# justinkay/coda

Hardware: AMD Instinct MI355X
Metric: acquisition_steps_per_sec (higher is better)
Workload: dtype fp32; 1 GPU; model=coda-eig, task=imagenet1k-scale, H_models=128, N_points=50000, C_classes=1000, prefilter_n=0, chunk_size=256, global_batch=50000, seq_len=1000, parallelism=single

## Files before the change

### coda_amd/ops/hip/pair.hip

```cpp

#include <climits>
#include <initializer_list>
#include <torch/extension.h>
#include <hip/hip_runtime.h>
#include <c10/hip/HIPStream.h>
#include <hip/hip_bfloat16.h>
#include "wave.h"

#define P_POINTS 256
#define BLOCK 256

namespace pairops {

typedef __bf16 bf16x8 __attribute__((ext_vector_type(8)));
typedef float f32x4 __attribute__((ext_vector_type(4)));
typedef _Float16 half4v __attribute__((ext_vector_type(4)));

__device__ __forceinline__ void
dsum_es_row(const _Float16* __restrict__ delta16,
            const float* __restrict__ dall,
            const int* __restrict__ pair_c,
            const int* __restrict__ pair_neg,
            const int* __restrict__ seg_off,
            const int* __restrict__ seg_h,
// ... 291 lines not shown
    for (int jt = 0; jt < JT; ++jt) {
        const int j = jt * 16 + row16;
        if (j >= twoH) continue;
        const int h = j >> 1, v = j & 1;
        const float mix = mixture0[h];
        const float pbb = pbest_before[(size_t)c * H + h];
#pragma unroll
        for (int r = 0; r < 4; ++r) {
            const int bit = (vmw[r][jt >> 2] >> (h & 31)) & 1;
            if (bit == v)
                pair_ent_acc(ent[r], mix, pic, acc[jt][r], inv[r], pbb);
        }
    }
#pragma unroll
    for (int r = 0; r < 4; ++r) {
        const float e = row16_reduce(ent[r]);
        if (row16 == 0) h_after[kbase + r] = e;
    }
    }
    (void)mstride;
}


template <int JT>
__global__ void __launch_bounds__(BLOCK2)
pair_gemm_pbn128_kernel(const hip_bfloat16* __restrict__ a16,
                        const hip_bfloat16* __restrict__ egw,
                        const unsigned* __restrict__ vmask,
                        const int* __restrict__ pair_c,
                        int W,
                        const int* __restrict__ grp_off,
                        const int* __restrict__ cls_grp_off,
                        const int* __restrict__ run_off,
                        const long long* __restrict__ y_t,
                        float* __restrict__ pm,
                        float* __restrict__ pinv,
                        int C, int H) {
    int g = blockIdx.x, a_row0 = 0;
    if (y_t != nullptr) {
        const long long y = y_t[0];
        if (y < 0 || y >= C) return;
        g += cls_grp_off[y];
        if (g >= cls_grp_off[y + 1]) return;
        a_row0 = run_off[y];
    }
    extern __shared__ char smem[];
    const int twoH = 2 * H;
    hip_bfloat16* b_lds = reinterpret_cast<hip_bfloat16*>(smem);

    const int t0 = grp_off[g], t1 = grp_off[g + 1];
    const int c = pair_c[t0 * 128];
    const int tid = threadIdx.x;
    const int wave = tid >> 6, lane = tid & 63;
    const int row16 = lane & 15;
    const int kgrp = lane >> 4;
    const hip_bfloat16* egw_c = egw + (size_t)c * twoH * P_POINTS;

    for (int t = tid; t < 2 * twoH; t += BLOCK2) {
        const int j = t >> 1, half = t & 1;
        const uint4* g = reinterpret_cast<const uint4*>(
            egw_c + (size_t)j * P_POINTS + half * 128);
        uint4* d = reinterpret_cast<uint4*>(
            reinterpret_cast<char*>(b_lds)
            + (size_t)j * BSTRIDE * 2 + half * 256);
#pragma unroll
        for (int i = 0; i < 16; ++i) d[i] = g[i];
    }
    __syncthreads();

    for (int tile = t0; tile < t1; ++tile) {
    const int k0 = tile * 128;
    f32x4 acc[JT];
#pragma unroll
    for (int jt = 0; jt < JT; ++jt) acc[jt] = {0.f, 0.f, 0.f, 0.f};

    const hip_bfloat16* arow =
        a16 + (size_t)(k0 - a_row0 + wave * 16 + row16) * P_POINTS;
#pragma unroll
    for (int kk = 0; kk < P_POINTS; kk += 32) {
        const bf16x8 afrag = *reinterpret_cast<const bf16x8*>(
            arow + kk + kgrp * 8);
#pragma unroll
        for (int jt = 0; jt < JT; ++jt) {
            const int j = jt * 16 + row16;
            bf16x8 bfrag = {};
            if (j < twoH)
                bfrag = *reinterpret_cast<const bf16x8*>(
                    b_lds + (size_t)j * BSTRIDE + kk + kgrp * 8);
            acc[jt] = __builtin_amdgcn_mfma_f32_16x16x32_bf16(
                afrag, bfrag, acc[jt], 0, 0, 0);
        }
    }

// ... 22 lines not shown
#pragma unroll
    for (int r = 0; r < 4; ++r)
        inv[r] = 1.0f / fmaxf(row16_reduce(tot[r]), 1e-30f);

#pragma unroll
    for (int jt = 0; jt < JT; ++jt) {
        const int j = jt * 16 + row16;
        if (j >= twoH) continue;
        const int h = j >> 1, v = j & 1;
#pragma unroll
        for (int r = 0; r < 4; ++r) {
            const int bit = (vmw[r][jt >> 2] >> (h & 31)) & 1;
            if (bit == v) pm[(size_t)(kbase + r) * H + h] = acc[jt][r];
        }
    }
#pragma unroll
    for (int r = 0; r < 4; ++r)
        if (row16 == 0) pinv[kbase + r] = inv[r];
    }
}


#define ECH 4

__global__ void __launch_bounds__(BLOCK)
pair_entropy_cached_kernel(const float* __restrict__ pm,
                           const float* __restrict__ pinv,
                           const unsigned* __restrict__ vmask,
                           const int* __restrict__ pair_c,
                           int W,
                           const float* __restrict__ pi_hat,
                           const float* __restrict__ pbest_before,
                           const float* __restrict__ mixture0,
                           float* __restrict__ h_after,
                           int H) {
    extern __shared__ char smem[];
    float* rows = reinterpret_cast<float*>(smem);
    float* mix_s = rows + 16 * H;
    float* pbb_s = mix_s + H;

    const int kb = blockIdx.x * (16 * ECH);
    const int c = pair_c[kb];
    const int tid = threadIdx.x;
    const int nv4 = 4 * H;
    const f32x4* g = reinterpret_cast<const f32x4*>(pm + (size_t)kb * H);
    const f32x4 zero4 = {0.f, 0.f, 0.f, 0.f};
    f32x4 nxt[3];
#pragma unroll
    for (int q = 0; q < 3; ++q)
        nxt[q] = tid + q * BLOCK < nv4 ? g[tid + q * BLOCK] : zero4;
    for (int h = tid; h < H; h += BLOCK) {
        mix_s[h] = mixture0[h];
        pbb_s[h] = pbest_before[(size_t)c * H + h];
    }
    const int pi = tid >> 4, l = tid & 15;
    const float pic = pi_hat[c];
    const float* row = rows + pi * H;
    const int twoH = 2 * H;
    const int JT = (twoH + 15) / 16;

#pragma unroll
    for (int ch = 0; ch < ECH; ++ch) {
        f32x4* d = reinterpret_cast<f32x4*>(rows);
#pragma unroll
        for (int q = 0; q < 3; ++q)
            if (tid + q * BLOCK < nv4) d[tid + q * BLOCK] = nxt[q];
        __syncthreads();
        if (ch + 1 < ECH) {
            const f32x4* gn = g + (size_t)(ch + 1) * nv4;
#pragma unroll
            for (int q = 0; q < 3; ++q)
                nxt[q] = tid + q * BLOCK < nv4 ? gn[tid + q * BLOCK]
                                               : zero4;
        }
        const int k = kb + ch * 16 + pi;
        const float inv = pinv[k];
        float ent = 0.f;
        unsigned vw = 0u;
        for (int jt = 0; jt < JT; ++jt) {
            const int j = jt * 16 + l;
            if ((jt & 3) == 0)
                vw = (jt >> 2) < W ? vmask[(size_t)k * W + (jt >> 2)] : 0u;
            if (j >= twoH) continue;
            const int h = j >> 1, v = j & 1;
            const int bit = (vw >> (h & 31)) & 1;
            if (bit == v)
                pair_ent_acc(ent, mix_s[h], pic, row[h], inv, pbb_s[h]);
        }
        const float e = row16_reduce(ent);
        if (l == 0) h_after[k] = e;
        __syncthreads();
    }
}

#define WSTRIDE 40

__global__ void __launch_bounds__(BLOCK)
pair_gemm_wide_kernel(const hip_bfloat16* __restrict__ a16,
                      const hip_bfloat16* __restrict__ egw,
                      const int* __restrict__ pair_c,
                      hip_bfloat16* __restrict__ mout,
                      int twoH) {
    extern __shared__ char smem[];
    hip_bfloat16* a_lds = reinterpret_cast<hip_bfloat16*>(smem);
    hip_bfloat16* b_lds = a_lds + 2 * 128 * WSTRIDE;

    const int k0 = blockIdx.x * 128;
    const int j0 = blockIdx.y * 128;
    const int c = pair_c[k0];
    const int tid = threadIdx.x;
    const int wave = tid >> 6, lane = tid & 63;
    const int row16 = lane & 15, kgrp = lane >> 4;
    const hip_bfloat16* egw_c = egw + (size_t)c * twoH * P_POINTS;
// ... 84 lines not shown
    float tot = 0.f;
    int i = 0;
    for (int h = lane; h < H; h += 64, ++i) {
        const int v = (vm[h >> 5] >> (h & 31)) & 1;
        val[i] = (float)mrow[2 * h + v];
        tot += val[i];
    }
    tot = wave_reduce_sum(tot);
    const float inv = 1.0f / fmaxf(tot, 1e-30f);
    const float pic = pi_hat[c];
    float ent = 0.f;
    i = 0;
    for (int h = lane; h < H; h += 64, ++i) {
        const float pb = val[i] * inv;
        const float mm = fmaxf(
            mixture0[h] + pic * (pb - pbest_before[(size_t)c * H + h]),
            1e-12f);
        ent += -mm * __log2f(mm);
    }
    ent = wave_reduce_sum(ent);
    if (lane == 0) h_after[k] = ent;
}

__global__ void __launch_bounds__(BLOCK)
pair_eig_finalize_kernel(const float* __restrict__ h_after,
                         const float* __restrict__ h_base,
                         const int* __restrict__ pair_c,
                         const int* __restrict__ cand_off,
                         const long long* __restrict__ cand_ck,
                         const long* __restrict__ cand_ids,
                         const float* __restrict__ adjusted,
                         const float* __restrict__ row_sums,
                         float H_before,
                         float* __restrict__ q,
                         int B, int C) {
    const int b = blockIdx.x * 4 + (threadIdx.x >> 6);
    if (b >= B) return;
    const int lane = threadIdx.x & 63;
    const long id = cand_ids[b];
    const float inv = 1.0f / fmaxf(row_sums[id], 1e-12f);
    const float* arow = adjusted + (size_t)id * C;
    float base = 0.f;
    int cc = lane * 4;
    for (; cc + 3 < C; cc += 256) {
        const float4 a = *reinterpret_cast<const float4*>(arow + cc);
        const float4 hb = *reinterpret_cast<const float4*>(h_base + cc);
        base += a.x * hb.x + a.y * hb.y + a.z * hb.z + a.w * hb.w;
    }
    for (; cc < C; ++cc) base += arow[cc] * h_base[cc];
    float corr = 0.f;
    const int s1 = cand_off[b + 1];
    for (int s = cand_off[b] + lane; s < s1; s += 64) {
        const long long pk = cand_ck[s];
        const int k = (int)(pk >> 32);
        const int c2 = (int)(pk & 0xffffffff);
        corr += arow[c2] * (h_after[k] - h_base[c2]);
    }
    (void)pair_c;
    const float tot = wave_reduce_sum(base + corr);
    if (lane == 0) q[b] = H_before - tot * inv;
}

__global__ void __launch_bounds__(BLOCK)
pair_entropy_wide_cls_kernel(const hip_bfloat16* __restrict__ m,
                             const int* __restrict__ cls,
                             const int* __restrict__ pair_b,
                             const int* __restrict__ pair_c,
                             const float* __restrict__ pi_hat,
                             const float* __restrict__ pbest_before,
                             const float* __restrict__ mixture0,
                             float* __restrict__ h_after,
                             int K, int H) {
    const int k = blockIdx.x * 4 + (threadIdx.x >> 6);
    if (k >= K) return;
    const int lane = threadIdx.x & 63;
    const int c = pair_c[k];
    const int b = pair_b[k];
    const hip_bfloat16* mrow = m + (size_t)k * 2 * H;

    float tot = 0.f;
    for (int h = lane; h < H; h += 64) {
        const int v = (b >= 0 && cls[(size_t)b * H + h] == c) ? 1 : 0;
        tot += (float)mrow[2 * h + v];
// ... 542 lines not shown
    TORCH_CHECK(grp.scalar_type() == torch::kInt32 && grp.is_contiguous()
                && grp.numel() >= 2, "grp must be the (G+1,) tile groups");
    const bool one_class = y_t_o.has_value();
    int nblk = grp.numel() - 1;
    const int* cgo = nullptr;
    const int* roff = nullptr;
    const long long* yp = nullptr;
    if (one_class) {
        TORCH_CHECK(cls_grp_off_o.has_value() && run_off_o.has_value(),
                    "one-class mode needs cls_grp_off and run_off");
        const torch::Tensor& y_t = *y_t_o;
        const torch::Tensor& cls_grp_off = *cls_grp_off_o;
        const torch::Tensor& run_off = *run_off_o;
        TORCH_CHECK(y_t.is_cuda() && y_t.scalar_type() == torch::kInt64
                    && y_t.numel() == 1, "y_t must be a (1,) int64 tensor");
        TORCH_CHECK(cls_grp_off.scalar_type() == torch::kInt32
                    && cls_grp_off.is_contiguous()
                    && cls_grp_off.numel() == C + 1
                    && run_off.scalar_type() == torch::kInt32
                    && run_off.is_contiguous()
                    && run_off.numel() == C + 1,
                    "cls_grp_off / run_off must be (C+1,) int32");
        TORCH_CHECK(max_grp >= 1 && max_grp <= nblk);
        nblk = (int)max_grp;
        cgo = cls_grp_off.data_ptr<int>();
        roff = run_off.data_ptr<int>();
        yp = reinterpret_cast<const long long*>(y_t.data_ptr<int64_t>());
    } else {
        TORCH_CHECK(a16.size(0) == K, "full build needs the (K, P) operand");
    }
    const size_t shmem = (size_t)2 * H * BSTRIDE * sizeof(hip_bfloat16);
    const int JT = (2 * H + 15) / 16;
    auto stream = c10::hip::getCurrentHIPStream();
    auto launch = [&](auto kern) {
        hipLaunchKernelGGL(kern, dim3(nblk), dim3(BLOCK2), shmem,
                           stream.stream(),
                           reinterpret_cast<const hip_bfloat16*>(
                               a16.data_ptr()),
                           reinterpret_cast<const hip_bfloat16*>(
                               egw.data_ptr()),
                           reinterpret_cast<const unsigned*>(
                               vmask.data_ptr<int>()),
                           pair_c.data_ptr<int>(), (int)vmask.size(1),
                           grp.data_ptr<int>(), cgo, roff, yp,
                           pm.data_ptr<float>(), pinv.data_ptr<float>(),
                           C, H);
    };
    if (JT <= 4) launch(pairops::pair_gemm_pbn128_kernel<4>);
    else if (JT <= 8) launch(pairops::pair_gemm_pbn128_kernel<8>);
    else if (JT <= 16) launch(pairops::pair_gemm_pbn128_kernel<16>);
    else launch(pairops::pair_gemm_pbn128_kernel<17>);
}

torch::Tensor pair_entropy_cached(torch::Tensor pm, torch::Tensor pinv,
                                  torch::Tensor vmask,
                                  torch::Tensor pair_c,
                                  torch::Tensor pi_hat,
                                  torch::Tensor pbest_before,
                                  torch::Tensor mixture0) {
    TORCH_CHECK(pm.is_cuda() && pm.dtype() == torch::kFloat32
                && pm.is_contiguous() && pm.dim() == 2);
    const int K = pm.size(0);
    const int H = pm.size(1);
    TORCH_CHECK(K % 128 == 0 && 2 * H <= 272,
                "pair cache covers the fused route only");
    TORCH_CHECK(pinv.is_contiguous() && pinv.numel() == K
                && pair_c.numel() == K && vmask.size(0) == K);
    TORCH_CHECK(mixture0.numel() == H && mixture0.is_contiguous()
                && pbest_before.is_contiguous()
                && pbest_before.size(1) == H
                && pi_hat.is_contiguous());
    auto h_after = torch::empty({K}, pi_hat.options());
    if (K == 0) return h_after;
    const size_t shmem = (size_t)18 * H * sizeof(float);
    auto stream = c10::hip::getCurrentHIPStream();
    hipLaunchKernelGGL(pairops::pair_entropy_cached_kernel,
                       dim3(K / (16 * ECH)), dim3(BLOCK), shmem,
                       stream.stream(),
                       pm.data_ptr<float>(), pinv.data_ptr<float>(),
                       reinterpret_cast<const unsigned*>(
                           vmask.data_ptr<int>()),
                       pair_c.data_ptr<int>(), (int)vmask.size(1),
                       pi_hat.data_ptr<float>(),
                       pbest_before.data_ptr<float>(),
                       mixture0.data_ptr<float>(),
                       h_after.data_ptr<float>(), H);
    return h_after;
}

torch::Tensor pair_eig_finalize(torch::Tensor h_after,
                                torch::Tensor h_base,
                                torch::Tensor pair_c,
                                torch::Tensor cand_off,
                                torch::Tensor cand_ck,
                                torch::Tensor cand_ids,
                                torch::Tensor adjusted,
                                torch::Tensor row_sums,
                                double H_before) {
    const int B = cand_ids.size(0);
    const int C = adjusted.size(1);
    TORCH_CHECK(h_base.is_contiguous() && h_base.size(0) == C);
    TORCH_CHECK(cand_ck.scalar_type() == torch::kInt64,
                "cand_ck must be the packed int64 hit table");
    TORCH_CHECK(cand_ids.is_contiguous() && cand_off.is_contiguous()
                && cand_ck.is_contiguous(),
                "finalize inputs must be contiguous");
    auto q = torch::empty({B}, adjusted.options());
    auto stream = c10::hip::getCurrentHIPStream();
    hipLaunchKernelGGL(pairops::pair_eig_finalize_kernel,
                       dim3((B + 3) / 4), dim3(BLOCK), 0, stream.stream(),
                       h_after.data_ptr<float>(),
                       h_base.data_ptr<float>(), pair_c.data_ptr<int>(),
                       cand_off.data_ptr<int>(),
                       reinterpret_cast<const long long*>(
                           cand_ck.data_ptr<int64_t>()),
                       cand_ids.data_ptr<long>(),
                       adjusted.data_ptr<float>(),
                       row_sums.data_ptr<float>(),
                       (float)H_before, q.data_ptr<float>(), B, C);
    return q;
}

void acq_select(torch::Tensor q0, torch::Tensor h0, torch::Tensor active,
                torch::Tensor qbuf, torch::Tensor out,
                torch::Tensor ties,
                c10::optional<torch::Tensor> topk_o,
                c10::optional<torch::Tensor> group_of_o,
                int64_t n_groups) {
    TORCH_CHECK(q0.is_cuda() && q0.dtype() == torch::kFloat32
                && q0.is_contiguous(), "q0 must be contiguous fp32");
    TORCH_CHECK(h0.dtype() == torch::kFloat32 && h0.numel() == 1);
    TORCH_CHECK(active.dtype() == torch::kBool && active.is_contiguous()
                && active.numel() == q0.numel());
    TORCH_CHECK(qbuf.dtype() == torch::kFloat32 && qbuf.is_contiguous()
                && qbuf.numel() == q0.numel());
    TORCH_CHECK(out.dtype() == torch::kFloat64 && out.is_contiguous()
                && out.numel() == 3);
    TORCH_CHECK(ties.dtype() == torch::kInt64 && ties.is_contiguous()
                && ties.numel() >= 2, "ties buffer too small");
    const int cap = ties.numel() - 1;
    const int B = q0.numel();
    const bool want_topk = topk_o.has_value() && topk_o->defined();
// ... 143 lines not shown
          pybind11::arg("vmask"), pybind11::arg("pair_c"),
          pybind11::arg("pi_hat"),
          pybind11::arg("pbest_before"), pybind11::arg("mixture0"),
          pybind11::arg("tile"), pybind11::arg("ablate") = 0,
          pybind11::arg("grp") = torch::Tensor());
    m.def("pair_gemm_entropy_cls", &pair_gemm_entropy_cls,
          "v3 wide-H pairing GEMM + cls-based entropy -> (K,)");
    m.def("pair_dsum_es_cls", &pair_dsum_es_cls,
          "pair A-operand of ONE class (id read on device) into the "
          "(max_run, P) scratch operand");
    m.def("pair_gemm_pbn", &pair_gemm_pbn,
          "pair-cache build (all groups) / one-class refresh: selected "
          "pairing masses pm (K, H) and inv (K,)",
          pybind11::arg("a16"), pybind11::arg("egw"),
          pybind11::arg("vmask"), pybind11::arg("pair_c"),
          pybind11::arg("grp"), pybind11::arg("pm"),
          pybind11::arg("pinv"),
          pybind11::arg("cls_grp_off") = pybind11::none(),
          pybind11::arg("run_off") = pybind11::none(),
          pybind11::arg("y_t") = pybind11::none(),
          pybind11::arg("max_grp") = 0);
    m.def("pair_entropy_cached", &pair_entropy_cached,
          "per-step entropy pass over the pair cache -> (K,), bit-equal "
          "to the fused 128-pair kernel");
    m.def("pair_eig_finalize", &pair_eig_finalize,
          "v3 per-candidate EIG assembly (deterministic) -> (B,)");
    m.def("acq_select", &acq_select,
          "fused acquisition epilogue: qbuf = active ? h0+q0 : -inf; "
          "out(f64[3]) = [masked max, first argmax, isclose tie count]; "
          "topk (K,) int64, when given, = the K best in rank order, one "
          "per group with group_of, -1 padded",
          pybind11::arg("q0"), pybind11::arg("h0"),
          pybind11::arg("active"), pybind11::arg("qbuf"),
          pybind11::arg("out"), pybind11::arg("ties"),
          pybind11::arg("topk") = pybind11::none(),
          pybind11::arg("group_of") = pybind11::none(),
          pybind11::arg("n_groups") = 0);
    m.def("mfma_probe", &mfma_probe,
          "16x16x32 bf16 MFMA fragment-layout probe");
}
```

### coda_amd/ops/hip/wave.h

```cpp
#pragma once

#include <hip/hip_runtime.h>

template <int CTRL, int ROW_MASK>
__device__ __forceinline__ int dpp_mov(int x) {
    return __builtin_amdgcn_update_dpp(0, x, CTRL, ROW_MASK, 0xf, true);
}

template <int CTRL, int ROW_MASK>
__device__ __forceinline__ float dpp_add(float x) {
    return x + __int_as_float(dpp_mov<CTRL, ROW_MASK>(__float_as_int(x)));
}

__device__ __forceinline__ float wave_inclusive_scan(float v) {
    v = dpp_add<0x111, 0xf>(v);
    v = dpp_add<0x112, 0xf>(v);
    v = dpp_add<0x114, 0xf>(v);
    v = dpp_add<0x118, 0xf>(v);
    v = dpp_add<0x142, 0xa>(v);
    v = dpp_add<0x143, 0xc>(v);
    return v;
}

__device__ __forceinline__ float wave_reduce_sum(float v) {
    return __int_as_float(__builtin_amdgcn_readlane(
        __float_as_int(wave_inclusive_scan(v)), 63));
}

__device__ __forceinline__ float row16_reduce(float v) {
    v = dpp_add<0x111, 0xf>(v);
    v = dpp_add<0x112, 0xf>(v);
    v = dpp_add<0x114, 0xf>(v);
    v = dpp_add<0x118, 0xf>(v);
    return __shfl(v, 15, 16);
}
```

### coda_amd/ops/pair.py

```python
from __future__ import annotations

from typing import NamedTuple, Optional

import torch

from .reference import EPS_PROB, PBEST_NUM_POINTS

PAIR_TILE = 16


def tile_for(H: int, B: int) -> int:
    return 128 if B >= 4096 else PAIR_TILE


class PairStructure(NamedTuple):
    cand_ids: torch.Tensor
    pair_b: torch.Tensor
    pair_c: torch.Tensor
    seg_off: torch.Tensor
    seg_h: torch.Tensor
    base_pos: torch.Tensor
    n_real: int
    tile: int
    cand_off: torch.Tensor = None
    cand_pairs: torch.Tensor = None
    vmask: torch.Tensor = None
    pair_neg: torch.Tensor = None
    cand_ck: torch.Tensor = None
    grp_off: torch.Tensor = None
    cls_grp_off: torch.Tensor = None
    run_off: torch.Tensor = None
    max_grp: int = 0
    max_run: int = 0

    @property
    def K(self) -> int:
        return self.pair_b.shape[0]


def build_pairs(cls_rows: torch.Tensor, cand_ids: torch.Tensor,
                C: int, tile: int = 0,
                with_vmask: bool = True,
                dedupe: bool = True) -> PairStructure:
    device = cls_rows.device
    B, H = cls_rows.shape
    tile = tile or tile_for(H, B)
    cls_l = cls_rows.long()
    keys = (cls_l * B + torch.arange(B, device=device).unsqueeze(1))
    flat = keys.reshape(-1)
    order = torch.argsort(flat, stable=True)
    sk = flat[order]
    is_new = torch.ones_like(sk, dtype=torch.bool)
    is_new[1:] = sk[1:] != sk[:-1]
    pair_key = sk[is_new]
    pr_c = pair_key // B
    pr_b = pair_key - pr_c * B
# ... 81 lines not shown
    h1 = entry_h[mask1]
    if bool(flip_real[reps_idx].any()):
        flipped_reps = reps_idx[flip_real[reps_idx]]
        pair_neg[pos[new_of_u[uid_of_real[flipped_reps]]]] = 1
        q_of_b = torch.full((B,), -1, dtype=torch.long, device=device)
        q_of_b[pr_b[flipped_reps]] = flipped_reps
        entry_b = pr_b[entry_pid]
        qb = q_of_b[entry_b]
        comp = (qb >= 0) & (entry_pid != qb)
        t2 = pos[new_of_u[uid_of_real[qb[comp]]]]
        h2 = entry_h[comp]
        tgt = torch.cat([t1, t2])
        hh = torch.cat([h1, h2])
    else:
        tgt, hh = t1, h1
    srt = torch.argsort(tgt * H + hh)
    seg_h = hh[srt].to(torch.int32)
    seg_len_k = torch.bincount(tgt, minlength=K)
    seg_off = torch.zeros(K + 1, dtype=torch.int32, device=device)
    seg_off[1:] = seg_len_k.cumsum(0).to(torch.int32)

    grp_off = None
    if tile == 128 and K % 128 == 0 and K > 0:
        GRP_MAX = 4
        tc = pair_c[::128]
        T = tc.numel()
        newc = torch.ones(T, dtype=torch.bool, device=device)
        newc[1:] = tc[1:] != tc[:-1]
        idx = torch.arange(T, device=device)
        run_start = idx[newc]
        run_id = newc.long().cumsum(0) - 1
        off_in_run = idx - run_start[run_id]
        gstart = newc | (off_in_run % GRP_MAX == 0)
        grp_off = torch.cat([
            idx[gstart].to(torch.int32),
            torch.tensor([T], dtype=torch.int32, device=device),
        ]).contiguous()
        grp_per_cls = torch.bincount(tc[gstart].long(), minlength=C)
        cls_grp_off = torch.zeros(C + 1, dtype=torch.int32, device=device)
        cls_grp_off[1:] = grp_per_cls.cumsum(0).to(torch.int32)
        per_class = dict(cls_grp_off=cls_grp_off,
                         run_off=run_off.to(torch.int32),
                         max_grp=int(grp_per_cls.max()),
                         max_run=int(run_len.max()))
    else:
        per_class = {}

    return PairStructure(**per_class,
                         cand_ids=cand_ids.long().contiguous(),
                         pair_b=pair_b,
                         pair_c=pair_c, seg_off=seg_off, seg_h=seg_h,
                         base_pos=run_off[:-1].clone(), n_real=K2,
                         tile=tile, cand_off=cand_off,
                         cand_pairs=cand_pairs, vmask=vmask,
                         pair_neg=pair_neg, grp_off=grp_off,
                         cand_ck=((cand_pairs.long() << 32)
                                  | pair_c[cand_pairs.long()].long())
                         .contiguous() if cand_pairs is not None
                         else None)


def pair_pbn(tables, ps: PairStructure, cls_rows: torch.Tensor,
             k0: int = 0, k1: Optional[int] = None) -> torch.Tensor:
    EG, delta, s_base, w = (tables.EG, tables.delta, tables.s_base,
                            tables.weights)
    C, H, _, P = EG.shape
    k1 = ps.K if k1 is None else k1
# ... 104 lines not shown
    if cache.pbn is not None:
        y = int(y)
        k0, k1 = int(ps.run_off[y]), int(ps.run_off[y + 1])
        cache.pbn[k0:k1] = pair_pbn(tables, ps, cls_rows, k0, k1)
        return
    import coda_amd.ops as O
    O._ext.pair_dsum_es_cls(tables.delta16, tables.dall, ps.pair_c,
                            ps.pair_neg, ps.seg_off, ps.seg_h,
                            ps.run_off, y, cache.a_run)
    O._ext.pair_gemm_pbn(cache.a_run, tables.egw, ps.vmask, ps.pair_c,
                         ps.grp_off, cache.pm, cache.pinv,
                         ps.cls_grp_off, ps.run_off, y, ps.max_grp)


def pair_cache_h_after(cache: PairCache, ps: PairStructure,
                       pi_hat: torch.Tensor, pbest_before: torch.Tensor,
                       mixture0: torch.Tensor) -> torch.Tensor:
    if cache.pbn is not None:
        return h_after_from_pbn(cache.pbn, ps, pi_hat, pbest_before,
                                mixture0)
    import coda_amd.ops as O
    return O._ext.pair_entropy_cached(
        cache.pm, cache.pinv, ps.vmask, ps.pair_c, pi_hat.contiguous(),
        pbest_before.contiguous(), mixture0.contiguous())


def eig_from_pairs(h_after: torch.Tensor, ps: PairStructure,
                   adjusted: torch.Tensor, row_sums: torch.Tensor,
                   H_before) -> torch.Tensor:
    N = adjusted.shape[0]
    h_base = h_after[ps.base_pos]
    inv_rs = 1.0 / row_sums.clamp_min(1e-12)
    base_n = (adjusted @ h_base) * inv_rs
    counts = (ps.cand_off[1:] - ps.cand_off[:-1]).long()
    ids = torch.repeat_interleave(ps.cand_ids, counts)
    k = ps.cand_pairs.long()
    c_v = ps.pair_c[k].long()
    pix = adjusted[ids, c_v] * inv_rs[ids]
    corr = torch.zeros(N, device=adjusted.device)
    corr.index_add_(0, ids, pix * (h_after[k] - h_base[c_v]))
    if torch.is_tensor(H_before):
        H_before = H_before.to(base_n.dtype)
    return H_before - base_n - corr


def _h_after_kernels(tables, ps: PairStructure, cls_rows, pbest_before,
                     pi_hat, mixture0) -> torch.Tensor:
# ... 76 lines not shown
```

### coda_amd/selectors/coda.py

```python
from __future__ import annotations

import random

import torch
from sortedcontainers import SortedList

from ..base import ModelSelector
from ..parallel import Comm, get_comm
from .. import ops
from ..ops import pair as pops
from ..ops import sharded as shops
from ..ops import table as tops
from ..util import DEBUG, _check, mirror_fits
from .pair_acq import PairAcquisition, tied_choice

import os
DEBUG_VIZ = os.environ.get("CODA_AMD_DEBUG_VIZ") == "1"

_ON_DEVICE = object()


def _warm_and_capture(body, read=None):
    side = torch.cuda.Stream()
    side.wait_stream(torch.cuda.current_stream())
# ... 111 lines not shown
        self.q_vals = []
        self.stochastic = False
        self.step = 0
        self.reset_derived_state()
        self.update_pi_hat()

    def reset_derived_state(self):
        self._tables = None
        self._tables_dirty = set()
        self._pair_acq = None
        self._posterior_version = 0
        self._pbest_rows_cache = (-1, None)
        self._drop_graphs()
        self._merged_acq = False
        self._g_idx = self._g_y = self._g_pi = self._g_rows = None
        self._alpha_g, self._beta_g = self._gather_global_betas()
        self._active_candidates = SortedList(
            i for i in self.unlabeled_idxs if self._disagreement_host[i])

    def _drop_graphs(self):
        self._label_graph = None
        self._acq_graph = None
        self._acq_pending = None

    def _gather_global_betas(self):
        if not self._replicated:
            return None, None
        a_l, b_l = ops.dirichlet_to_beta(self.dirichlets)
        sizes = self.comm.shard_sizes(self.H)
        order = self.comm.unshard_order(self.H).to(self.device)
        return tuple(self.comm.all_gather_cat(
            t, dim=0, sizes=sizes)[order].contiguous() for t in (a_l, b_l))

    @classmethod
    def from_args(cls, dataset, args, comm=None):
        return cls(dataset,
                   prefilter_n=args.prefilter_n,
                   alpha=args.alpha,
                   learning_rate=args.learning_rate,
                   multiplier=args.multiplier,
                   disable_diag_prior=args.no_diag_prior,
                   q=args.q,
                   comm=comm,
                   chunk_size=getattr(args, "chunk_size", 100),
                   pi_hat_precision=getattr(args, "pi_hat_precision",
                                            "auto"))
# ... 216 lines not shown
                    hsizes=self.comm.shard_sizes(self.H))
            elif self.comm.is_distributed:
                eig = shops.eig_chunk_sharded(
                    alpha_cc, beta_cc, chunk_classes, pbest_before,
                    self.pi_hat, pi_xi, mixture0, H_before, self.comm,
                    num_points=self.num_points)
            elif tables is not None:
                eig = tops.eig_chunk_table(
                    tables, chunk_classes, pbest_before, self.pi_hat,
                    pi_xi, mixture0, H_before)
            else:
                eig = ops.eig_chunk(
                    alpha_cc, beta_cc, chunk_classes, pbest_before,
                    self.pi_hat, pi_xi, mixture0, H_before,
                    num_points=self.num_points)
            eig_chunks.append(eig)

        return torch.cat(eig_chunks), candidate_ids

    def _acq_body(self):
        acq = self._pair_acq
        rows, pi = self._g_rows, self._g_pi
        mixture0, H0 = ops.mixture_entropy(rows, pi)
        h_after = None if acq.cache is None else pops.pair_cache_h_after(
            acq.cache, acq.ps, pi, rows, mixture0)
        q0 = pops.eig_pairs(self._tables, acq.ps, acq.cls_rows, rows, pi,
                            mixture0, None, self._adjusted, self._row_sums,
                            h_after=h_after)
        ops._ext.acq_select(q0.contiguous(), H0.reshape(1).contiguous(),
                            acq.active, acq.qbuf, acq.out, acq.ties,
                            *acq.topk_args())

    def _acq_result(self):
        idx, q, tied = self._pair_acq.result()
        self.stochastic |= tied
        return idx, q

    def _acq_eligible(self) -> bool:
        return (self.q == "eig" and self._pair_acq is not None
                and self._pair_acq.ps.vmask is not None
                and not DEBUG_VIZ
                and not (self.prefilter_n
                         and len(self._active_candidates)
                         > self.prefilter_n))

    def _graphed_acquire(self, read=None):
# ... 130 lines not shown

    def _graphed_add_label(self, idx: int, y: int):
        first = self._label_graph is None
        if first:
            self._sync_pair_cache()
            self._acq_graph = None
            self._g_idx = torch.zeros(1, dtype=torch.long,
                                      device=self.device)
            self._g_y = torch.zeros(1, dtype=torch.long, device=self.device)
            self._g_pi = torch.empty_like(self.pi_hat)
            self._g_rows = self._pbest_rows_before().clone().contiguous()
            self._merged_acq = self._acq_eligible()
        self._g_idx.fill_(idx)
        self._g_y.fill_(y)
        pending = _ON_DEVICE
        if first:
            def body():
                self._graph_label_update()
                if self._merged_acq:
                    self._acq_body()

            self._label_graph, pending = _warm_and_capture(
                body, self._acq_result if self._merged_acq else None)
        else:
            self._label_graph.replay()
        self.pi_hat = self._g_pi
        self._pi_xi_cache = None
        self._pbest_rows_cache = (self._posterior_version + 1,
                                  self._g_rows)
        self._acq_pending = pending if self._merged_acq else None

    def _eager_add_label(self, idx: int, y: int):
        y_t = torch.tensor([y], dtype=torch.long, device=self.device)
        self.pi_hat = self._posterior_update(
            y_t, self.classes[:, idx].contiguous())
        self._pi_xi_cache = None
        if self._replicated:
            hit = self.classes_global[:, idx].long() == y
            self._alpha_g[:, y] += self.update_strength * hit.float()
            self._beta_g[:, y] += self.update_strength * (~hit).float()
        self._tables_dirty.add(y)
        ver, cached = self._pbest_rows_cache
        if (cached is not None and ver == self._posterior_version
                and (self._replicated or not self.comm.is_distributed)):
            if self._replicated:
                a_col = self._alpha_g[:, y].contiguous()
                b_col = self._beta_g[:, y].contiguous()
            else:
# ... 2 lines not shown
                b_col = (row.sum(-1) - a_col).contiguous()
            rows = cached.clone()
            rows[y] = ops.pbest_from_beta(
                a_col.unsqueeze(0), b_col.unsqueeze(0),
                self.num_points)[0]
            self._pbest_rows_cache = (self._posterior_version + 1, rows)

    def add_label(self, idx, true_class, selection_prob):
        idx, y = int(idx), int(true_class)
        self._deactivate(idx)
        if (self._use_label_graph and self._tables is not None
                and not self._tables_dirty):
            self._graphed_add_label(idx, y)
        else:
            self._eager_add_label(idx, y)
        self._posterior_version += 1
        self.labeled_idxs.append(idx)
        self.labels.append(y)
        self.q_vals.append(selection_prob)
        self.unlabeled_idxs.remove(idx)

    def _deactivate(self, idx: int):
        self._acq_pending = None
        try:
            self._active_candidates.remove(idx)
        except ValueError:
            pass
        if self._pair_acq is not None:
            self._pair_acq.deactivate(idx)

    def skip(self, idx):
        idx = int(idx)
        if idx in self.unlabeled_idxs:
            self.unlabeled_idxs.remove(idx)
        self._deactivate(idx)

    def get_pbest(self):
        rows = self._pbest_rows_before()
        marg_local = ops.mixture_entropy(rows, self.pi_hat)[0]
        if self.comm.is_distributed and not self._replicated:
            gathered = self.comm.all_gather_cat(marg_local, dim=0)
            pbest = gathered[self.comm.unshard_order(self.H).to(gathered.device)]
        else:
            pbest = marg_local
        if DEBUG:
            _check(pbest, "Pbest")
        return pbest

    def get_best_model_prediction(self):
        pbest = self.get_pbest()
        if DEBUG_VIZ:
            from ..util import plot_bar
            from .. import tracking
            try:
                tracking.log_image(plot_bar(pbest, title="PBest"),
                                   key="PBest", step=self.step)
            except RuntimeError:
                pass
        self.step += 1
        return torch.argmax(pbest)
```

Measured before the change: 2326 steps/s.

## Split pbn128 groups across blocks, skip pad chunks, retile entropy and finalize kernels

The per-class pair GEMM now launches PBN_GRP_TILES blocks per group, each taking a strided subset of tiles, to raise parallelism. The cached entropy kernel moves to 8 lanes per row with 32 rows per chunk and padded LDS rows. It also skips all-pad chunks via run_off/run_live, filling them from one base-row entropy. The finalize kernel becomes grid-strided with h_base staged in LDS and prefetching of the next candidate. get_pbest reuses the mixture entropy computed inside the captured acquisition graph instead of recomputing it. Splitting groups repeats the B-operand LDS load per block, and the pad-skip assumes pad rows share one entropy value.

Result: faster. 2636 steps/s (median of 6 runs) (+13.4%).

```diff
diff --git a/coda_amd/ops/hip/pair.hip b/coda_amd/ops/hip/pair.hip
--- a/coda_amd/ops/hip/pair.hip
+++ b/coda_amd/ops/hip/pair.hip
@@ -1,4 +1,5 @@
 
+#include <algorithm>
 #include <climits>
 #include <initializer_list>
 #include <torch/extension.h>
@@ -337,6 +338,8 @@
 }
 
 
+#define PBN_GRP_TILES 4
+
 template <int JT>
 __global__ void __launch_bounds__(BLOCK2)
 pair_gemm_pbn128_kernel(const hip_bfloat16* __restrict__ a16,
@@ -351,19 +354,27 @@
                         float* __restrict__ pm,
                         float* __restrict__ pinv,
                         int C, int H) {
-    int g = blockIdx.x, a_row0 = 0;
+    int g = blockIdx.x, a_row0 = 0, tsel = -1;
     if (y_t != nullptr) {
         const long long y = y_t[0];
         if (y < 0 || y >= C) return;
-        g += cls_grp_off[y];
+        g = cls_grp_off[y] + (int)(blockIdx.x / PBN_GRP_TILES);
         if (g >= cls_grp_off[y + 1]) return;
+        tsel = (int)(blockIdx.x % PBN_GRP_TILES);
         a_row0 = run_off[y];
     }
     extern __shared__ char smem[];
     const int twoH = 2 * H;
     hip_bfloat16* b_lds = reinterpret_cast<hip_bfloat16*>(smem);
 
-    const int t0 = grp_off[g], t1 = grp_off[g + 1];
+    int t0 = grp_off[g];
+    const int t1 = grp_off[g + 1];
+    int tstep = 1;
+    if (tsel >= 0) {
+        t0 += tsel;
+        if (t0 >= t1) return;
+        tstep = PBN_GRP_TILES;
+    }
     const int c = pair_c[t0 * 128];
     const int tid = threadIdx.x;
     const int wave = tid >> 6, lane = tid & 63;
@@ -383,7 +394,7 @@
     }
     __syncthreads();
 
-    for (int tile = t0; tile < t1; ++tile) {
+    for (int tile = t0; tile < t1; tile += tstep) {
     const int k0 = tile * 128;
     f32x4 acc[JT];
 #pragma unroll
@@ -452,6 +463,34 @@
 
 
 #define ECH 4
+#define ENQ 5
+#define EWMAX 5
+
+__host__ __device__ __forceinline__ int pair_ent_stride(int H) {
+    return ((H + 55) / 64) * 64 + 8;
+}
+
+__device__ __forceinline__ float
+pair_ent_row8(const float* row, const float* mix_s, const float* pbb_s,
+              const unsigned (&vw)[EWMAX], float inv, float pic, int m,
+              int H) {
+    float even = 0.f, odd = 0.f;
+#pragma unroll
+    for (int w = 0; w < EWMAX; ++w) {
+#pragma unroll
+        for (int t = 0; t < 4; ++t) {
+            const int h = (4 * w + t) * 8 + m;
+            if (h < H) {
+                const bool bit = (vw[w] >> (h & 31)) & 1;
+                float sel = bit ? odd : even;
+                pair_ent_acc(sel, mix_s[h], pic, row[h], inv, pbb_s[h]);
+                even = bit ? even : sel;
+                odd = bit ? sel : odd;
+            }
+        }
+    }
+    return row8_reduce_last(odd + even);
+}
 
 __global__ void __launch_bounds__(BLOCK)
 pair_entropy_cached_kernel(const float* __restrict__ pm,
@@ -462,63 +501,108 @@
                            const float* __restrict__ pi_hat,
                            const float* __restrict__ pbest_before,
                            const float* __restrict__ mixture0,
+                           const int* __restrict__ run_off,
+                           const int* __restrict__ run_live,
                            float* __restrict__ h_after,
                            int H) {
     extern __shared__ char smem[];
+    const int stride = pair_ent_stride(H);
     float* rows = reinterpret_cast<float*>(smem);
-    float* mix_s = rows + 16 * H;
+    float* mix_s = rows + 32 * stride;
     float* pbb_s = mix_s + H;
-
-    const int kb = blockIdx.x * (16 * ECH);
+    float* brow = pbb_s + H;
+    float* bval = brow + H;
+
+    const int kb = blockIdx.x * (32 * ECH);
     const int c = pair_c[kb];
     const int tid = threadIdx.x;
-    const int nv4 = 4 * H;
+    const int pi = tid >> 3, m = tid & 7;
+    int nlive = ECH, kbase = 0;
+    if (run_live != nullptr) {
+        kbase = run_off[c];
+        const int rem = kbase + run_live[c] - kb;
+        nlive = rem <= 0 ? 0 : (rem >= 32 * ECH ? ECH : (rem + 31) >> 5);
+    }
+
+    const int nv4 = 8 * H;
     const f32x4* g = reinterpret_cast<const f32x4*>(pm + (size_t)kb * H);
     const f32x4 zero4 = {0.f, 0.f, 0.f, 0.f};
-    f32x4 nxt[3];
-#pragma unroll
-    for (int q = 0; q < 3; ++q)
-        nxt[q] = tid + q * BLOCK < nv4 ? g[tid + q * BLOCK] : zero4;
+    f32x4 nxt[ENQ];
+    if (nlive > 0) {
+#pragma unroll
+        for (int q = 0; q < ENQ; ++q)
+            nxt[q] = tid + q * BLOCK < nv4 ? g[tid + q * BLOCK] : zero4;
+    }
     for (int h = tid; h < H; h += BLOCK) {
         mix_s[h] = mixture0[h];
         pbb_s[h] = pbest_before[(size_t)c * H + h];
-    }
-    const int pi = tid >> 4, l = tid & 15;
+        if (nlive < ECH) brow[h] = pm[(size_t)kbase * H + h];
+    }
     const float pic = pi_hat[c];
-    const float* row = rows + pi * H;
-    const int twoH = 2 * H;
-    const int JT = (twoH + 15) / 16;
-
-#pragma unroll
-    for (int ch = 0; ch < ECH; ++ch) {
-        f32x4* d = reinterpret_cast<f32x4*>(rows);
-#pragma unroll
-        for (int q = 0; q < 3; ++q)
-            if (tid + q * BLOCK < nv4) d[tid + q * BLOCK] = nxt[q];
+    int drow[ENQ], dcol[ENQ];
+#pragma unroll
+    for (int q = 0; q < ENQ; ++q) {
+        const int e = 4 * (tid + q * BLOCK);
+        drow[q] = e / H;
+        dcol[q] = e - drow[q] * H;
+    }
+
+    if (nlive < ECH) {
         __syncthreads();
-        if (ch + 1 < ECH) {
+        if (pi == 0) {
+            unsigned vw[EWMAX];
+#pragma unroll
+            for (int w = 0; w < EWMAX; ++w)
+                vw[w] = w < W ? vmask[(size_t)kbase * W + w] : 0u;
+            const float e = pair_ent_row8(brow, mix_s, pbb_s, vw,
+                                          pinv[kbase], pic, m, H);
+            if (m == 7) bval[0] = e;
+        }
+        __syncthreads();
+        const float e = bval[0];
+        for (int r = nlive * 32 + tid; r < 32 * ECH; r += BLOCK)
+            h_after[kb + r] = e;
+        if (nlive == 0) return;
+    }
+
+#pragma unroll 1
+    for (int ch = 0; ch < nlive; ++ch) {
+        const int k = kb + ch * 32 + pi;
+        unsigned vw[EWMAX];
+#pragma unroll
+        for (int w = 0; w < EWMAX; ++w)
+            vw[w] = w < W ? vmask[(size_t)k * W + w] : 0u;
+        const float inv = pinv[k];
+        if ((H & 3) == 0) {
+#pragma unroll
+            for (int q = 0; q < ENQ; ++q)
+                if (tid + q * BLOCK < nv4)
+                    *reinterpret_cast<f32x4*>(
+                        rows + drow[q] * stride + dcol[q]) = nxt[q];
+        } else {
+#pragma unroll
+            for (int q = 0; q < ENQ; ++q)
+                if (tid + q * BLOCK < nv4) {
+                    int r = drow[q], cc = dcol[q];
+#pragma unroll
+                    for (int i = 0; i < 4; ++i) {
+                        while (cc >= H) { cc -= H; ++r; }
+                        rows[r * stride + cc] = nxt[q][i];
+                        ++cc;
+                    }
+                }
+        }
+        __syncthreads();
+        if (ch + 1 < nlive) {
             const f32x4* gn = g + (size_t)(ch + 1) * nv4;
 #pragma unroll
-            for (int q = 0; q < 3; ++q)
+            for (int q = 0; q < ENQ; ++q)
                 nxt[q] = tid + q * BLOCK < nv4 ? gn[tid + q * BLOCK]
                                                : zero4;
         }
-        const int k = kb + ch * 16 + pi;
-        const float inv = pinv[k];
-        float ent = 0.f;
-        unsigned vw = 0u;
-        for (int jt = 0; jt < JT; ++jt) {
-            const int j = jt * 16 + l;
-            if ((jt & 3) == 0)
-                vw = (jt >> 2) < W ? vmask[(size_t)k * W + (jt >> 2)] : 0u;
-            if (j >= twoH) continue;
-            const int h = j >> 1, v = j & 1;
-            const int bit = (vw >> (h & 31)) & 1;
-            if (bit == v)
-                pair_ent_acc(ent, mix_s[h], pic, row[h], inv, pbb_s[h]);
-        }
-        const float e = row16_reduce(ent);
-        if (l == 0) h_after[k] = e;
+        const float e = pair_ent_row8(rows + pi * stride, mix_s, pbb_s, vw,
+                                      inv, pic, m, H);
+        if (m == 7) h_after[k] = e;
         __syncthreads();
     }
 }
@@ -649,10 +733,13 @@
     if (lane == 0) h_after[k] = ent;
 }
 
+#define FIN_MAX_BLOCKS 2048
+#define FIN_LDS_MAX_C 8192
+
+template <bool HB_LDS, bool VEC>
 __global__ void __launch_bounds__(BLOCK)
 pair_eig_finalize_kernel(const float* __restrict__ h_after,
                          const float* __restrict__ h_base,
-                         const int* __restrict__ pair_c,
                          const int* __restrict__ cand_off,
                          const long long* __restrict__ cand_ck,
                          const long* __restrict__ cand_ids,
@@ -660,32 +747,105 @@
                          const float* __restrict__ row_sums,
                          float H_before,
                          float* __restrict__ q,
-                         int B, int C) {
-    const int b = blockIdx.x * 4 + (threadIdx.x >> 6);
+                         int B, int C, int nhits) {
+    extern __shared__ char smem[];
+    float* hb_s = reinterpret_cast<float*>(smem);
+    if constexpr (HB_LDS) {
+        for (int i = threadIdx.x; i < C; i += BLOCK) hb_s[i] = h_base[i];
+        __syncthreads();
+    }
+    auto hb1 = [&](int i) -> float {
+        if constexpr (HB_LDS) return hb_s[i]; else return h_base[i];
+    };
+    auto hb4 = [&](int i) -> f32x4 {
+        if constexpr (HB_LDS)
+            return *reinterpret_cast<const f32x4*>(hb_s + i);
+        else
+            return *reinterpret_cast<const f32x4*>(h_base + i);
+    };
+
+    const int lane = threadIdx.x & 63;
+    const int wave = __builtin_amdgcn_readfirstlane(threadIdx.x >> 6);
+    const int stride = gridDim.x * 4;
+    int b = blockIdx.x * 4 + wave;
     if (b >= B) return;
-    const int lane = threadIdx.x & 63;
-    const long id = cand_ids[b];
-    const float inv = 1.0f / fmaxf(row_sums[id], 1e-12f);
-    const float* arow = adjusted + (size_t)id * C;
-    float base = 0.f;
-    int cc = lane * 4;
-    for (; cc + 3 < C; cc += 256) {
-        const float4 a = *reinterpret_cast<const float4*>(arow + cc);
-        const float4 hb = *reinterpret_cast<const float4*>(h_base + cc);
-        base += a.x * hb.x + a.y * hb.y + a.z * hb.z + a.w * hb.w;
-    }
-    for (; cc < C; ++cc) base += arow[cc] * h_base[cc];
-    float corr = 0.f;
-    const int s1 = cand_off[b + 1];
-    for (int s = cand_off[b] + lane; s < s1; s += 64) {
-        const long long pk = cand_ck[s];
-        const int k = (int)(pk >> 32);
+    const int n4 = C - 3 > 4 * lane ? (C - 3 - 4 * lane + 255) / 256 : 0;
+    const int n4w = C > 3 ? (C - 3 + 255) / 256 : 0;
+    const int cvec = C - 4;
+    const int cvec_hb = cvec & ~3;
+    const int nh1 = nhits - 1;
+
+    long id = cand_ids[b];
+    int s0 = cand_off[b], s1 = cand_off[b + 1];
+    for (;;) {
+        const int s = s0 + lane;
+        const bool hit = s < s1;
+        const long long pk0 = cand_ck[min(hit ? s : s0, nh1)];
+        long long pk = hit ? pk0 : 0;
+        const float rs = row_sums[id];
+        const float* arow = adjusted + (size_t)id * C;
+        const int bn = b + stride;
+        const int bnc = min(bn, B - 1);
+        const long idn = cand_ids[bnc];
+        const int s0n = cand_off[bnc], s1n = cand_off[bnc + 1];
+
+        float base = 0.f;
+        f32x4 a[4], hb[4];
+        if constexpr (VEC) {
+#pragma unroll
+            for (int j = 0; j < 4; ++j)
+                a[j] = *reinterpret_cast<const f32x4*>(
+                    arow + min(lane * 4 + j * 256, cvec));
+        }
         const int c2 = (int)(pk & 0xffffffff);
-        corr += arow[c2] * (h_after[k] - h_base[c2]);
-    }
-    (void)pair_c;
-    const float tot = wave_reduce_sum(base + corr);
-    if (lane == 0) q[b] = H_before - tot * inv;
+        const float ga = arow[c2];
+        const float gh = h_after[(int)(pk >> 32)];
+        const float ghb = hb1(c2);
+        if constexpr (VEC) {
+#pragma unroll
+            for (int j = 0; j < 4; ++j)
+                hb[j] = hb4(min(lane * 4 + j * 256, cvec_hb));
+#pragma unroll
+            for (int j = 0; j < 4; ++j) {
+                const float nb = base
+                    + (a[j][0] * hb[j][0] + a[j][1] * hb[j][1]
+                       + a[j][2] * hb[j][2] + a[j][3] * hb[j][3]);
+                base = j < n4 ? nb : base;
+            }
+            for (int i0 = 4; i0 < n4w; i0 += 4) {
+#pragma unroll
+                for (int j = 0; j < 4; ++j)
+                    a[j] = *reinterpret_cast<const f32x4*>(
+                        arow + min(lane * 4 + (i0 + j) * 256, cvec));
+#pragma unroll
+                for (int j = 0; j < 4; ++j)
+                    hb[j] = hb4(min(lane * 4 + (i0 + j) * 256, cvec_hb));
+#pragma unroll
+                for (int j = 0; j < 4; ++j) {
+                    const float nb = base
+                        + (a[j][0] * hb[j][0] + a[j][1] * hb[j][1]
+                           + a[j][2] * hb[j][2] + a[j][3] * hb[j][3]);
+                    base = i0 + j < n4 ? nb : base;
+                }
+            }
+        }
+        for (int cc = lane * 4 + n4 * 256; cc < C; ++cc)
+            base += arow[cc] * hb1(cc);
+
+        const float c0 = 0.f + ga * (gh - ghb);
+        float corr = hit ? c0 : 0.f;
+        for (int s2 = s + 64; s2 < s1; s2 += 64) {
+            pk = cand_ck[s2];
+            const int k = (int)(pk >> 32);
+            const int cx = (int)(pk & 0xffffffff);
+            corr += arow[cx] * (h_after[k] - hb1(cx));
+        }
+        const float inv = 1.0f / fmaxf(rs, 1e-12f);
+        const float tot = wave_reduce_sum(base + corr);
+        if (lane == 0) q[b] = H_before - tot * inv;
+        if (bn >= B) break;
+        b = bn; id = idn; s0 = s0n; s1 = s1n;
+    }
 }
 
 __global__ void __launch_bounds__(BLOCK)
@@ -1274,7 +1434,7 @@
                     && run_off.numel() == C + 1,
                     "cls_grp_off / run_off must be (C+1,) int32");
         TORCH_CHECK(max_grp >= 1 && max_grp <= nblk);
-        nblk = (int)max_grp;
+        nblk = (int)max_grp * PBN_GRP_TILES;
         cgo = cls_grp_off.data_ptr<int>();
         roff = run_off.data_ptr<int>();
         yp = reinterpret_cast<const long long*>(y_t.data_ptr<int64_t>());
@@ -1309,7 +1469,9 @@
                                   torch::Tensor pair_c,
                                   torch::Tensor pi_hat,
                                   torch::Tensor pbest_before,
-                                  torch::Tensor mixture0) {
+                                  torch::Tensor mixture0,
+                                  c10::optional<torch::Tensor> run_off_o,
+                                  c10::optional<torch::Tensor> run_live_o) {
     TORCH_CHECK(pm.is_cuda() && pm.dtype() == torch::kFloat32
                 && pm.is_contiguous() && pm.dim() == 2);
     const int K = pm.size(0);
@@ -1318,16 +1480,35 @@
                 "pair cache covers the fused route only");
     TORCH_CHECK(pinv.is_contiguous() && pinv.numel() == K
                 && pair_c.numel() == K && vmask.size(0) == K);
+    TORCH_CHECK(vmask.is_contiguous() && vmask.size(1) <= EWMAX);
     TORCH_CHECK(mixture0.numel() == H && mixture0.is_contiguous()
                 && pbest_before.is_contiguous()
                 && pbest_before.size(1) == H
                 && pi_hat.is_contiguous());
+    TORCH_CHECK(run_off_o.has_value() == run_live_o.has_value(),
+                "run_off and run_live go together");
+    const int* roff = nullptr;
+    const int* rlive = nullptr;
+    if (run_off_o.has_value()) {
+        const torch::Tensor& run_off = *run_off_o;
+        const torch::Tensor& run_live = *run_live_o;
+        const int64_t C = pbest_before.size(0);
+        TORCH_CHECK(run_off.is_cuda() && run_live.is_cuda()
+                    && run_off.scalar_type() == torch::kInt32
+                    && run_live.scalar_type() == torch::kInt32
+                    && run_off.is_contiguous() && run_live.is_contiguous()
+                    && run_off.numel() == C + 1 && run_live.numel() == C,
+                    "run_off (C+1,) / run_live (C,) must be int32");
+        roff = run_off.data_ptr<int>();
+        rlive = run_live.data_ptr<int>();
+    }
     auto h_after = torch::empty({K}, pi_hat.options());
     if (K == 0) return h_after;
-    const size_t shmem = (size_t)18 * H * sizeof(float);
+    const size_t shmem = ((size_t)32 * pairops::pair_ent_stride(H)
+                          + 3 * H + 1) * sizeof(float);
     auto stream = c10::hip::getCurrentHIPStream();
     hipLaunchKernelGGL(pairops::pair_entropy_cached_kernel,
-                       dim3(K / (16 * ECH)), dim3(BLOCK), shmem,
+                       dim3(K / (32 * ECH)), dim3(BLOCK), shmem,
                        stream.stream(),
                        pm.data_ptr<float>(), pinv.data_ptr<float>(),
                        reinterpret_cast<const unsigned*>(
@@ -1335,7 +1516,7 @@
                        pair_c.data_ptr<int>(), (int)vmask.size(1),
                        pi_hat.data_ptr<float>(),
                        pbest_before.data_ptr<float>(),
-                       mixture0.data_ptr<float>(),
+                       mixture0.data_ptr<float>(), roff, rlive,
                        h_after.data_ptr<float>(), H);
     return h_after;
 }
@@ -1358,18 +1539,37 @@
                 && cand_ck.is_contiguous(),
                 "finalize inputs must be contiguous");
     auto q = torch::empty({B}, adjusted.options());
+    if (B == 0) return q;
+    (void)pair_c;
+    TORCH_CHECK(cand_off.numel() == B + 1 && cand_ck.numel() < INT_MAX);
+    TORCH_CHECK(h_after.numel() >= 1 && C >= 1,
+                "finalize needs at least one pair and one class");
+    const int nhits = cand_ck.numel() ? (int)cand_ck.numel() : 1;
+    const long long* ckp = cand_ck.numel()
+        ? reinterpret_cast<const long long*>(cand_ck.data_ptr<int64_t>())
+        : reinterpret_cast<const long long*>(cand_ids.data_ptr<int64_t>());
     auto stream = c10::hip::getCurrentHIPStream();
-    hipLaunchKernelGGL(pairops::pair_eig_finalize_kernel,
-                       dim3((B + 3) / 4), dim3(BLOCK), 0, stream.stream(),
-                       h_after.data_ptr<float>(),
-                       h_base.data_ptr<float>(), pair_c.data_ptr<int>(),
-                       cand_off.data_ptr<int>(),
-                       reinterpret_cast<const long long*>(
-                           cand_ck.data_ptr<int64_t>()),
-                       cand_ids.data_ptr<long>(),
-                       adjusted.data_ptr<float>(),
-                       row_sums.data_ptr<float>(),
-                       (float)H_before, q.data_ptr<float>(), B, C);
+    const int nblk = std::min((B + 3) / 4, FIN_MAX_BLOCKS);
+    auto launch = [&](auto kern, size_t shmem) {
+        hipLaunchKernelGGL(kern, dim3(nblk), dim3(BLOCK), shmem,
+                           stream.stream(),
+                           h_after.data_ptr<float>(),
+                           h_base.data_ptr<float>(),
+                           cand_off.data_ptr<int>(),
+                           ckp, cand_ids.data_ptr<long>(),
+                           adjusted.data_ptr<float>(),
+                           row_sums.data_ptr<float>(),
+                           (float)H_before, q.data_ptr<float>(), B, C,
+                           nhits);
+    };
+    if (C < 4)
+        launch(pairops::pair_eig_finalize_kernel<true, false>,
+               (size_t)C * sizeof(float));
+    else if (C <= FIN_LDS_MAX_C)
+        launch(pairops::pair_eig_finalize_kernel<true, true>,
+               (size_t)C * sizeof(float));
+    else
+        launch(pairops::pair_eig_finalize_kernel<false, true>, 0);
     return q;
 }
 
@@ -1559,7 +1759,14 @@
           pybind11::arg("max_grp") = 0);
     m.def("pair_entropy_cached", &pair_entropy_cached,
           "per-step entropy pass over the pair cache -> (K,), bit-equal "
-          "to the fused 128-pair kernel");
+          "to the fused 128-pair kernel; run_off + run_live skip the "
+          "all-pad chunks",
+          pybind11::arg("pm"), pybind11::arg("pinv"),
+          pybind11::arg("vmask"), pybind11::arg("pair_c"),
+          pybind11::arg("pi_hat"), pybind11::arg("pbest_before"),
+          pybind11::arg("mixture0"),
+          pybind11::arg("run_off") = pybind11::none(),
+          pybind11::arg("run_live") = pybind11::none());
     m.def("pair_eig_finalize", &pair_eig_finalize,
           "v3 per-candidate EIG assembly (deterministic) -> (B,)");
     m.def("acq_select", &acq_select,
diff --git a/coda_amd/ops/hip/wave.h b/coda_amd/ops/hip/wave.h
--- a/coda_amd/ops/hip/wave.h
+++ b/coda_amd/ops/hip/wave.h
@@ -34,3 +34,10 @@
     v = dpp_add<0x118, 0xf>(v);
     return __shfl(v, 15, 16);
 }
+
+__device__ __forceinline__ float row8_reduce_last(float v) {
+    v = dpp_add<0x111, 0xf>(v);
+    v = dpp_add<0x112, 0xf>(v);
+    v = dpp_add<0x114, 0xf>(v);
+    return v;
+}
diff --git a/coda_amd/ops/pair.py b/coda_amd/ops/pair.py
--- a/coda_amd/ops/pair.py
+++ b/coda_amd/ops/pair.py
@@ -11,6 +11,9 @@
 
 def tile_for(H: int, B: int) -> int:
     return 128 if B >= 4096 else PAIR_TILE
+
+
+GRP_MAX = 4
 
 
 class PairStructure(NamedTuple):
@@ -32,6 +35,7 @@
     run_off: torch.Tensor = None
     max_grp: int = 0
     max_run: int = 0
+    run_live: torch.Tensor = None
 
     @property
     def K(self) -> int:
@@ -159,7 +163,6 @@
 
     grp_off = None
     if tile == 128 and K % 128 == 0 and K > 0:
-        GRP_MAX = 4
         tc = pair_c[::128]
         T = tc.numel()
         newc = torch.ones(T, dtype=torch.bool, device=device)
@@ -179,7 +182,8 @@
         per_class = dict(cls_grp_off=cls_grp_off,
                          run_off=run_off.to(torch.int32),
                          max_grp=int(grp_per_cls.max()),
-                         max_run=int(run_len.max()))
+                         max_run=int(run_len.max()),
+                         run_live=(class_counts + 1).to(torch.int32))
     else:
         per_class = {}
 
@@ -330,7 +334,8 @@
     import coda_amd.ops as O
     return O._ext.pair_entropy_cached(
         cache.pm, cache.pinv, ps.vmask, ps.pair_c, pi_hat.contiguous(),
-        pbest_before.contiguous(), mixture0.contiguous())
+        pbest_before.contiguous(), mixture0.contiguous(),
+        ps.run_off, ps.run_live)
 
 
 def eig_from_pairs(h_after: torch.Tensor, ps: PairStructure,
diff --git a/coda_amd/selectors/coda.py b/coda_amd/selectors/coda.py
--- a/coda_amd/selectors/coda.py
+++ b/coda_amd/selectors/coda.py
@@ -157,6 +157,8 @@
         self._label_graph = None
         self._acq_graph = None
         self._acq_pending = None
+        self._mixture_cache = (-1, None)
+        self._acq_mixture = self._label_mixture = None
 
     def _gather_global_betas(self):
         if not self._replicated:
@@ -419,6 +421,7 @@
         acq = self._pair_acq
         rows, pi = self._g_rows, self._g_pi
         mixture0, H0 = ops.mixture_entropy(rows, pi)
+        self._acq_mixture = mixture0
         h_after = None if acq.cache is None else pops.pair_cache_h_after(
             acq.cache, acq.ps, pi, rows, mixture0)
         q0 = pops.eig_pairs(self._tables, acq.ps, acq.cls_rows, rows, pi,
@@ -595,8 +598,13 @@
 
             self._label_graph, pending = _warm_and_capture(
                 body, self._acq_result if self._merged_acq else None)
+            self._label_mixture = (self._acq_mixture if self._merged_acq
+                                   else None)
         else:
             self._label_graph.replay()
+            if self._label_mixture is not None:
+                self._mixture_cache = (self._posterior_version + 1,
+                                       self._label_mixture)
         self.pi_hat = self._g_pi
         self._pi_xi_cache = None
         self._pbest_rows_cache = (self._posterior_version + 1,
@@ -645,6 +653,7 @@
 
     def _deactivate(self, idx: int):
         self._acq_pending = None
+        self._mixture_cache = (-1, None)
         try:
             self._active_candidates.remove(idx)
         except ValueError:
@@ -659,8 +668,13 @@
         self._deactivate(idx)
 
     def get_pbest(self):
-        rows = self._pbest_rows_before()
-        marg_local = ops.mixture_entropy(rows, self.pi_hat)[0]
+        ver, mix = self._mixture_cache
+        if (mix is not None and ver == self._posterior_version
+                and not self.comm.is_distributed):
+            marg_local = mix.clone()
+        else:
+            rows = self._pbest_rows_before()
+            marg_local = ops.mixture_entropy(rows, self.pi_hat)[0]
         if self.comm.is_distributed and not self._replicated:
             gathered = self.comm.all_gather_cat(marg_local, dim=0)
             pbest = gathered[self.comm.unshard_order(self.H).to(gathered.device)]
```
